# dgrzech/ir-sgmcmc

Measured on AMD Instinct MI355X. Metric: SG-MCMC transitions/sec (full _SGLD_transition), higher is better.
Workload: dtype f32; 1 GPU; 256^3 synthetic pair, SVF_3D 12 steps, GMM(K=4)/LCC(s=1) + virtual decimation, RegLoss_L2 w=1.4, Sobolev s=3, uniform noise 0.1, SGLD lr 0.4, Philox noise; init=identity, chains=1, parallelism=1 independent chain(s)

## Files before the change

### include/irsgmcmc.h

```cpp
#ifndef IRSGMCMC_H
#define IRSGMCMC_H

#include <stddef.h>
#include <stdint.h>

#ifdef __cplusplus
extern "C" {
#endif
#pragma GCC visibility push(default)

#define IRS_MAX_COMPONENTS 8
#define IRS_MAX_CHAINS 8
#define IRS_MAX_HALF_WIDTH 4
#define IRS_MAX_LABELS 64

enum { IRS_DATA_GMM_LCC = 0, IRS_DATA_SSD = 1 };
enum { IRS_REG_L2 = 0, IRS_REG_LOGNORMAL = 1, IRS_REG_STUDENT = 2, IRS_REG_LOGNORMAL_L2 = 3 };


int irs_perturb_smooth(const float* v, const float* sigma, const float* eps, float tau, const float* kernel, int s,
                       int C, int D, int H, int W, float* tmp, float* out, uint64_t seed, uint64_t iteration,
                       void* stream);

int irs_svf_exp_fwd(const float* v, float* steps, float* transformation, float* displacement, int no_steps, int C,
                    int D, int H, int W, void* stream);

int irs_svf_exp_bwd(const float* v, const float* steps, const float* g_last, float* scratch, float* g_v, int no_steps,
                    int C, int D, int H, int W, void* stream);

int irs_ffd_up(const float* v_cp, float* dense, float* tmp, int C, int D, int H, int W, int c0, int c1, int c2,
               void* stream);
int irs_ffd_adjoint(const float* g_dense, float* g_cp, float* tmp, int C, int D, int H, int W, int c0, int c1, int c2,
                    void* stream);

int irs_warp_fwd(const float* im, int Cim, const float* d_last, const float* unif, float alpha, float* warped, int C,
                 int D, int H, int W, uint64_t seed, uint64_t iteration, void* stream);
int irs_warp_bwd(const float* im, int Cim, const float* d_last, const float* unif, float alpha, const float* g_warped,
                 float* g_d, int C, int D, int H, int W, uint64_t seed, uint64_t iteration, void* stream);
int irs_warp_transformation(const float* im, int Cim, const float* transformation, float* warped, int C, int D, int H,
                            int W, void* stream);
int irs_warp_nearest_u8(const uint8_t* seg, int Cim, const float* transformation, uint8_t* out, int C, int D, int H,
                        int W, void* stream);
int irs_warp_nearest_i16(const int16_t* seg, int Cim, const float* transformation, int16_t* out, int C, int D, int H,
                         int W, void* stream);

int irs_lcc_normalise(const float* im, float* out, float* sigma_out, int s, int C, int D, int H, int W, void* stream);
int irs_lcc_map_fwd(const float* fhat, int Cf, const float* warped, float* z, float* sigma_m, int s, int C, int D,
                    int H, int W, void* stream);
int irs_lcc_map_bwd(const float* fhat, int Cf, const float* z, const float* sigma_m, const float* g_z, float* g_warped,
                    int s, int C, int D, int H, int W, void* stream);

int irs_reg_energy(const float* v, double* y_out, double* partials, int C, int D, int H, int W, void* stream);
size_t irs_reduce_scratch_doubles(void);
int irs_gradient_operator(const float* v, float* nabla, int transformation, int C, int D, int H, int W, void* stream);
int irs_log_det_jacobian(const float* transformation, float* log_det, long long* nan_count, int C, int D, int H, int W,
                         void* stream);

int irs_label_boxes(const int16_t* seg_fixed, int Cf, const int16_t* seg_moving, const int32_t* labels, int n_labels,
                    int32_t* boxes, int C, int D, int H, int W, void* stream);
// ... 211 lines not shown
```

### ir_sgmcmc_amd/_lib.py

```python
import ctypes as C
import os

import torch

_HERE = os.path.dirname(os.path.abspath(__file__))
LIB_PATH = os.environ.get('IRS_LIB') or os.path.join(_HERE, 'csrc', 'libirsgmcmc.so')

IRS_MAX_COMPONENTS = 8
IRS_MAX_CHAINS = 8
IRS_MAX_HALF_WIDTH = 4
IRS_MAX_LABELS = 64
IRS_DATA_GMM_LCC, IRS_DATA_SSD = 0, 1
IRS_REG_L2, IRS_REG_LOGNORMAL, IRS_REG_STUDENT, IRS_REG_LOGNORMAL_L2 = 0, 1, 2, 3


class IrsConfig(C.Structure):
    _fields_ = [
        ('dims', C.c_int32 * 3), ('cps', C.c_int32 * 3), ('no_chains', C.c_int32), ('no_steps', C.c_int32),
        ('sobolev_s', C.c_int32), ('sobolev_kernel', C.c_float * (2 * IRS_MAX_HALF_WIDTH + 1)),
        ('lr', C.c_float), ('uniform_alpha', C.c_float), ('virtual_decimation', C.c_int32),
        ('data_loss', C.c_int32), ('lcc_s', C.c_int32), ('gmm_components', C.c_int32), ('ssd_sigma', C.c_float),
        ('gmm_lr_log_std', C.c_float), ('gmm_lr_logits', C.c_float), ('gmm_lr_decay', C.c_float),
        ('adam_beta1', C.c_float), ('adam_beta2', C.c_float), ('adam_eps', C.c_float),
        ('scale_prior_loc', C.c_float), ('scale_prior_scale', C.c_float),
# ... 64 lines not shown
    _fields_ = [(n, C.c_int32) for n in ('kind', 'stage', 'k', 'lo0', 'hi0', 'lo1', 'hi1', 'in0', 'in1', 'reach', 'out', 'width', 'id')]


IRS_OP_LAUNCH, IRS_OP_EXCHANGE, IRS_OP_ALLREDUCE, IRS_OP_WAIT = range(4)
(IRS_SG_PERTURB, IRS_SG_COPY_V, IRS_SG_SMOOTH, IRS_SG_ENERGY, IRS_SG_EXP_FWD, IRS_SG_OUTPUTS, IRS_SG_WARP, IRS_SG_RESIDUAL, IRS_SG_STATS,
 IRS_SG_DATA_BWD, IRS_SG_WARP_BWD, IRS_SG_EXP_BWD, IRS_SG_UPDATE, IRS_SG_FFD_UP, IRS_SG_FFD_ADJ) = range(15)
IRS_SG_CHAIN_SCALAR, IRS_SG_REG_SCALAR, IRS_SG_FINALIZE = 32, 33, 34
(IRS_SB_V, IRS_SB_NOISY, IRS_SB_VS, IRS_SB_WARPED, IRS_SB_Z, IRS_SB_GM, IRS_SB_GRAD_A, IRS_SB_GRAD_B, IRS_SB_DENSE, IRS_SB_GRAD_C) = range(10)
IRS_SB_STEP0 = 16
IRS_COMM_ID_BYTES = 128
EXCHANGE_FN = C.CFUNCTYPE(C.c_int, C.c_void_p, C.POINTER(IrsXfer), C.c_int, C.c_void_p)
ALLREDUCE_FN = C.CFUNCTYPE(C.c_int, C.c_void_p, C.c_void_p, C.c_size_t, C.c_int, C.c_void_p)

_P, _I, _F, _U64 = C.c_void_p, C.c_int, C.c_float, C.c_uint64
_I32P = C.POINTER(C.c_int32)

SIGNATURES = {
    'irs_perturb_smooth': [_P, _P, _P, _F, _P, _I, _I, _I, _I, _I, _P, _P, _U64, _U64, _P],
    'irs_svf_exp_fwd': [_P, _P, _P, _P, _I, _I, _I, _I, _I, _P],
    'irs_svf_exp_bwd': [_P, _P, _P, _P, _P, _I, _I, _I, _I, _I, _P],
    'irs_ffd_up': [_P, _P, _P, _I, _I, _I, _I, _I, _I, _I, _P],
    'irs_ffd_adjoint': [_P, _P, _P, _I, _I, _I, _I, _I, _I, _I, _P],
    'irs_warp_fwd': [_P, _I, _P, _P, _F, _P, _I, _I, _I, _I, _U64, _U64, _P],
    'irs_warp_bwd': [_P, _I, _P, _P, _F, _P, _P, _I, _I, _I, _I, _U64, _U64, _P],
    'irs_warp_transformation': [_P, _I, _P, _P, _I, _I, _I, _I, _P],
    'irs_warp_nearest_u8': [_P, _I, _P, _P, _I, _I, _I, _I, _P],
    'irs_warp_nearest_i16': [_P, _I, _P, _P, _I, _I, _I, _I, _P],
    'irs_lcc_normalise': [_P, _P, _P, _I, _I, _I, _I, _I, _P],
    'irs_lcc_map_fwd': [_P, _I, _P, _P, _P, _I, _I, _I, _I, _I, _P],
    'irs_lcc_map_bwd': [_P, _I, _P, _P, _P, _P, _I, _I, _I, _I, _I, _P],
    'irs_reg_energy': [_P, _P, _P, _I, _I, _I, _I, _P],
    'irs_reduce_scratch_doubles': [],
    'irs_gradient_operator': [_P, _P, _I, _I, _I, _I, _I, _P],
    'irs_log_det_jacobian': [_P, _P, _P, _I, _I, _I, _I, _P],
    'irs_label_boxes': [_P, _I, _P, _I32P, _I, _P, _I, _I, _I, _I, _P],
    'irs_surface_distance_workspace': [_I32P, _I, _I, _I, _I, C.POINTER(C.c_size_t)],
    'irs_label_surface_distance': [_P, _I, _P, _I32P, _I, C.POINTER(C.c_float), _I32P, _P, C.c_size_t, _P, _P, _I, _I, _I, _I,
                                   _P],
    'irs_chain_moments_update': [_P, _I, _I, _I, _I, _I, _I, _P, _P, _P],
    'irs_split_rhat_workspace': [_I, _I, _I, _I, C.POINTER(C.c_size_t)],
    'irs_split_rhat': [_P, _P, _I, _I, _P, C.c_float, C.c_float, _P, _P, _P, C.c_size_t, _I, _I, _I, _P],
    'irs_chain_variogram_update': [_P, _I, _I, _I, _I, _I, _I, _P, _P, _P],
    'irs_split_ess_workspace': [_I, _I, _I, _I, C.POINTER(C.c_size_t)],
    'irs_split_ess': [_P, _P, _P, _I, _I, _I, _P, C.c_float, _P, _P, _P, _P, C.c_size_t, _I, _I, _I, _P],
    'irs_create': [C.POINTER(IrsConfig), C.POINTER(_P)],
    'irs_destroy': [_P],
# ... 90 lines not shown
```

### ir_sgmcmc_amd/csrc/api.hip

```cpp
#include <math.h>
#include <stdarg.h>
#include <stdio.h>
#include <stdlib.h>
#include <string.h>

#include <algorithm>
#include <mutex>
#include <new>
#include <vector>

#include "comm.h"
#include "ctx.h"

using namespace irs;

namespace irs {
thread_local char g_err[512] = "";

int fail(const char* fmt, ...) {
    va_list ap;
    va_start(ap, fmt);
    vsnprintf(g_err, sizeof(g_err), fmt, ap);
    va_end(ap);
    return 1;
// ... 4 lines not shown

static int env_or(const char* name, int dflt) {
    const char* v = getenv(name);
    return v && *v ? atoi(v) : dflt;
}

static Knobs knobs_from_env() {
    Knobs k;
    k.predict_variants = env_or("IRS_PREDICT_VARIANTS", k.predict_variants);
    k.run_ahead = env_or("IRS_RUN_AHEAD", k.run_ahead);
    k.fuse_warp_bwd = env_or("IRS_FUSE_WARP_BWD", k.fuse_warp_bwd);
    k.energy_in_update = env_or("IRS_ENERGY_IN_UPDATE", k.energy_in_update);
    k.fuse_noise = env_or("IRS_FUSE_NOISE", k.fuse_noise);
    k.recover = env_or("IRS_RECOVER", k.recover);
    k.fwd_rows1 = env_or("IRS_FWD_ROWS1", k.fwd_rows1);
    k.coarse_box = env_or("IRS_COARSE_BOX", k.coarse_box);
    k.lds_from = env_or("IRS_LDS_FROM", k.lds_from);
    k.seg_fit = env_or("IRS_SEG_FIT", k.seg_fit);
    k.fwd_pf = env_or("IRS_FWD_PF", k.fwd_pf);
    k.fwd_z2 = env_or("IRS_FWD_Z2", k.fwd_z2);
    k.tile_box = env_or("IRS_TILE_BOX", k.tile_box);
    k.fwd_r2_rows1 = env_or("IRS_FWD_R2_ROWS1", k.fwd_r2_rows1);
    k.ps_rows = env_or("IRS_PS_ROWS", k.ps_rows);
    const char* tile = getenv("IRS_SOBOLEV_TILE");
    if (tile && *tile) k.sobolev_tile = tile[0] == 'b' ? 2 : (tile[0] == 's' ? 1 : atoi(tile));
    k.march_seg = env_or("IRS_MARCH_SEG", k.march_seg);
    k.march_seg_fwd = env_or("IRS_MARCH_SEG_FWD", k.march_seg_fwd);
    k.swz_run = env_or("IRS_SWZ_RUN", k.swz_run);
    k.seg_min_blocks = env_or("IRS_SEG_MIN_BLOCKS", k.seg_min_blocks);
    k.seg_min_len = env_or("IRS_SEG_MIN_LEN", k.seg_min_len);
    k.sobolev_seg = env_or("IRS_SOBOLEV_SEG", k.sobolev_seg);
    k.lcc_seg = env_or("IRS_LCC_SEG", k.lcc_seg);
    k.stats_seg = env_or("IRS_STATS_SEG", k.stats_seg);
    k.update_seg = env_or("IRS_UPDATE_SEG", k.update_seg);
    k.slab_split = env_or("IRS_SLAB_SPLIT", k.slab_split);
    k.slab_buffers = env_or("IRS_SLAB_BUFFERS", k.slab_buffers);
    k.slab_exact = env_or("IRS_SLAB_EXACT", k.slab_exact);
    k.slab_force_h = env_or("IRS_SLAB_FORCE_H", k.slab_force_h);
    k.launch_log = env_or("IRS_LAUNCH_LOG", k.launch_log);
    k.chain_overlap = env_or("IRS_CHAIN_OVERLAP", k.chain_overlap);
    k.data_batch = env_or("IRS_DATA_BATCH", k.data_batch);
    return k;
}

Knobs& global_knobs() {
    static Knobs k = knobs_from_env();
// ... 20 lines not shown
            (double)steps / (double)(steps - run_in > 0 ? steps - run_in : 1));
}

static int g_live_contexts = 0;
void context_born() { ++g_live_contexts; }
void context_gone() { --g_live_contexts; }

enum { KN_CTX = 0, KN_GLOBAL = 1, KN_LAYOUT = 2 };

int knob_set(Knobs& k, const char* name, int value, bool on_context) {
    struct Entry {
        const char* name;
        int Knobs::*field;
        int scope;
    };
    static const Entry table[] = {
        {"predict_variants", &Knobs::predict_variants, KN_CTX}, {"run_ahead", &Knobs::run_ahead, KN_CTX}, {"fuse_warp_bwd", &Knobs::fuse_warp_bwd, KN_CTX},
        {"energy_in_update", &Knobs::energy_in_update, KN_CTX}, {"fuse_noise", &Knobs::fuse_noise, KN_CTX}, {"recover", &Knobs::recover, KN_CTX},
        {"chain_overlap", &Knobs::chain_overlap, KN_CTX}, {"data_batch", &Knobs::data_batch, KN_CTX}, {"slab_split", &Knobs::slab_split, KN_CTX}, {"slab_buffers", &Knobs::slab_buffers, KN_CTX}, {"slab_exact", &Knobs::slab_exact, KN_CTX}, {"slab_force_h", &Knobs::slab_force_h, KN_CTX},
        {"fwd_rows1", &Knobs::fwd_rows1, KN_GLOBAL}, {"coarse_box", &Knobs::coarse_box, KN_GLOBAL}, {"lds_from", &Knobs::lds_from, KN_GLOBAL},
        {"fwd_pf", &Knobs::fwd_pf, KN_GLOBAL}, {"fwd_z2", &Knobs::fwd_z2, KN_GLOBAL}, {"tile_box", &Knobs::tile_box, KN_GLOBAL}, {"fwd_r2_rows1", &Knobs::fwd_r2_rows1, KN_GLOBAL}, {"sobolev_tile", &Knobs::sobolev_tile, KN_GLOBAL},
        {"march_seg", &Knobs::march_seg, KN_GLOBAL}, {"march_seg_fwd", &Knobs::march_seg_fwd, KN_GLOBAL}, {"swz_run", &Knobs::swz_run, KN_GLOBAL},
        {"sobolev_seg", &Knobs::sobolev_seg, KN_GLOBAL}, {"ps_rows", &Knobs::ps_rows, KN_GLOBAL}, {"launch_log", &Knobs::launch_log, KN_GLOBAL},
        {"seg_fit", &Knobs::seg_fit, KN_LAYOUT}, {"seg_min_blocks", &Knobs::seg_min_blocks, KN_LAYOUT}, {"seg_min_len", &Knobs::seg_min_len, KN_LAYOUT},
        {"lcc_seg", &Knobs::lcc_seg, KN_LAYOUT}, {"stats_seg", &Knobs::stats_seg, KN_LAYOUT}, {"update_seg", &Knobs::update_seg, KN_LAYOUT},
    };
    if (!name) return fail("irs_option_set: null name");
    for (const Entry& e : table)
        if (!strcmp(e.name, name)) {
            if (on_context && e.scope != KN_CTX)
                return fail("irs_option_set: '%s' is a process-wide switch (the launchers read it at every launch): set it with ctx == NULL", name);
            if (!on_context && e.scope == KN_LAYOUT && g_live_contexts > 0 && k.*(e.field) != value)
                return fail("irs_option_set: '%s' sizes the partial-sum layout of a context at creation; %d context(s) are alive -- set it before irs_create", name, g_live_contexts);
            k.*(e.field) = value;
            return 0;
        }
    return fail("irs_option_set: unknown option '%s'", name);
}
}

namespace {

bool dims_ok(int C, int D, int H, int W) {
    return C >= 1 && D >= 2 && H >= 2 && W >= 2 && (int64_t)D * H * W < ((int64_t)1 << 30);
}

// ... 179 lines not shown
               void* stream) {
    if (!v_cp || !dense || !tmp || !dims_ok(C, D, H, W) || c0 < 1 || c1 < 1 || c2 < 1 || c0 > 8 || c1 > 8 || c2 > 8)
        return fail("irs_ffd_up: bad arguments");
    const Vol vol = make_vol(D, H, W);
    const int G[3] = {control_points(D, c0), control_points(H, c1), control_points(W, c2)};
    const SplineTaps spl[3] = {make_spline(c0), make_spline(c1), make_spline(c2)};
    ffd_up(v_cp, dense, tmp, C, vol, G, spl, (hipStream_t)stream);
    LAUNCH_CHECK();
    return 0;
}

int irs_ffd_adjoint(const float* g_dense, float* g_cp, float* tmp, int C, int D, int H, int W, int c0, int c1, int c2,
                    void* stream) {
    if (!g_dense || !g_cp || !tmp || !dims_ok(C, D, H, W) || c0 < 1 || c1 < 1 || c2 < 1 || c0 > 8 || c1 > 8 || c2 > 8)
        return fail("irs_ffd_adjoint: bad arguments");
    const Vol vol = make_vol(D, H, W);
    const int G[3] = {control_points(D, c0), control_points(H, c1), control_points(W, c2)};
    const SplineTaps spl[3] = {make_spline(c0), make_spline(c1), make_spline(c2)};
    ffd_adjoint(g_dense, g_cp, tmp, C, vol, G, spl, (hipStream_t)stream);
    LAUNCH_CHECK();
    return 0;
}

int irs_warp_fwd(const float* im, int Cim, const float* d_last, const float* unif, float alpha, float* warped, int C,
                 int D, int H, int W, uint64_t seed, uint64_t iteration, void* stream) {
    if (!im || !d_last || !warped || !dims_ok(C, D, H, W) || (Cim != 1 && Cim != C)) return fail("irs_warp_fwd: bad arguments");
    hipStream_t st = (hipStream_t)stream;
    const Vol vol = make_vol(D, H, W);
    Lin lin;
    if (cached_lin(D, H, W, st, &lin)) return fail("irs_warp_fwd: identity grid allocation failed");
    launch_warp_fwd(im, Cim == 1 ? 0 : vol.V, d_last, unif, alpha, warped, nullptr, 0, C, vol, lin, seed, iteration, nullptr, st);
    LAUNCH_CHECK();
    return 0;
}

int irs_warp_bwd(const float* im, int Cim, const float* d_last, const float* unif, float alpha, const float* g_warped,
                 float* g_d, int C, int D, int H, int W, uint64_t seed, uint64_t iteration, void* stream) {
    if (!im || !d_last || !g_warped || !g_d || !dims_ok(C, D, H, W) || (Cim != 1 && Cim != C))
        return fail("irs_warp_bwd: bad arguments");
    hipStream_t st = (hipStream_t)stream;
    const Vol vol = make_vol(D, H, W);
    Lin lin;
    if (cached_lin(D, H, W, st, &lin)) return fail("irs_warp_bwd: identity grid allocation failed");
    launch_warp_bwd(im, Cim == 1 ? 0 : vol.V, d_last, unif, alpha, g_warped, g_d, C, vol, lin, seed, iteration, nullptr, st);
    LAUNCH_CHECK();
    return 0;
// ... 590 lines not shown
            launch_sobolev_march(c->tmpA, vs, c->sob, C * 3, c->volv, have_dmax0 ? c->dmax : nullptr, cfg.no_steps, st);
        }
    }
    const float* dense = vs;
    if (c->ffd) {
        const int G[3] = {c->volv.D, c->volv.H, c->volv.W};
        ffd_up(vs, c->dense, c->tmpA, C, c->vol, G, c->spl, st);
        dense = c->dense;
    }
    if (timed) HIP_TRY(hipEventRecord(c->ev[1], st));
    const int64_t field = (int64_t)c->C * 3 * c->vol.V;
    const Lin lin = c->lin.lin();
    if (!have_dmax0) launch_field_absmax(dense, true, cfg.no_steps, c->dmax, C, c->vol, st);
    for (int k = 0; k < cfg.no_steps; ++k) {
        const float* in = k == 0 ? dense : c->steps + (int64_t)(k - 1) * field;
        float* out = c->steps + (int64_t)k * field;
        launch_exp_step_fwd_march(in, out, k == 0, cfg.no_steps, C, c->vol, lin, c->dmax + (int64_t)k * c->C * 4,
                                  c->dmax + (int64_t)(k + 1) * c->C * 4, predicted_small(c, k), fwd_lay(c, k), st);
    }
    if (timed) HIP_TRY(hipEventRecord(c->ev[2], st));
    const float* d_last = c->steps + (int64_t)(cfg.no_steps - 1) * field;
    const float alpha = with_jitter ? cfg.uniform_alpha : 0.0f;
    launch_warp_fwd(io->moving_im, io->moving_chains == 1 ? 0 : c->vol.V, d_last, io->unif, alpha, warped, gradm, 1, C, c->vol, lin,
                    cfg.seed, 0, it, st);
    if (cfg.data_loss == IRS_DATA_GMM_LCC)
        launch_lcc_fwd_march(c->fhat, c->fhat_chains == 1 ? 0 : c->vol.V, warped, z, c->sigM, cfg.lcc_s, C, c->vol, st);
    else
        launch_residual_ssd(io->fixed_im, io->fixed_chains == 1 ? 0 : c->vol.V, warped, z, C, c->vol, st);
    LAUNCH_CHECK();
    return 0;
}

int irs_gmm_init(irs_ctx* c, const irs_io* io, const float* v_sample, int warm_up, void* stream) {
    if (check_io(c, io, "irs_gmm_init")) return 1;
    if (c->cfg.data_loss != IRS_DATA_GMM_LCC) return 0;
    hipStream_t st = (hipStream_t)stream;
    const size_t bytes = (size_t)3 * c->volv.V * sizeof(float);
    if (v_sample) HIP_TRY(hipMemcpyAsync(c->tmpB, v_sample, bytes, hipMemcpyDeviceToDevice, st));
    else HIP_TRY(hipMemsetAsync(c->tmpB, 0, bytes, st));
    if (forward_pass(c, io, c->tmpB, false, false, c->vs, c->warped, c->z, nullptr, 1, st, 0)) return 1;
    launch_masked_moments(c->z, io->mask, c->stat_partials, c->vol, st);
    launch_gmm_init_from_moments(c->state, c->stat_partials, stats_blocks(c->vol), c->dcfg, st);
    launch_stats(c->cfg.virtual_decimation, c->z, io->mask, c->state, c->stat_partials, c->vol, st, c->dcfg.K);
    launch_chain_scalar(c->state, c->stat_partials, stats_blocks(c->vol), 0, 1, c->dcfg, st);
    for (int i = 0; i < warm_up; ++i) {
        launch_stats(0, c->z, io->mask, c->state, c->stat_partials, c->vol, st, c->dcfg.K);
        launch_chain_scalar(c->state, c->stat_partials, stats_blocks(c->vol), 0, 2, c->dcfg, st);
// ... 233 lines not shown
```

### ir_sgmcmc_amd/csrc/common.h

```cpp
#pragma once
#include <hip/hip_runtime.h>
#include <math.h>
#include <stdint.h>
#include <stdlib.h>

#include "../../include/irsgmcmc.h"

namespace irs {

constexpr int kBlock = 256;
constexpr int kWave = 64;
constexpr int kMaxPartialBlocks = 2048;

struct Vol {
    int D, H, W;
    int64_t V;
    int z0, nz;
    int z0b, nzb;
    int64_t Vg;
};

__host__ __device__ inline Vol make_vol(int D, int H, int W) {
    return Vol{D, H, W, (int64_t)D * H * W, 0, D, 0, 0, (int64_t)D * H * W};
}
// ... 43 lines not shown
    int run_ahead = 2;
    int fuse_warp_bwd = 1;
    int energy_in_update = 1;
    int fuse_noise = 1;
    int recover = 1;
    int fwd_rows1 = -1;
    int lds_from = 3;
    int fwd_r2_rows1 = 1;
    int fwd_z2 = 0;
    int tile_box = 1;
    int fwd_pf = 2;
    int seg_fit = 1;
    int coarse_box = 1;
    int sobolev_tile = 0;
    int ps_rows = 0;
    int march_seg = 0, march_seg_fwd = 0, swz_run = -1, seg_min_blocks = 0, seg_min_len = 0;
    int sobolev_seg = 0, lcc_seg = 0, stats_seg = 0, update_seg = 0;
    int slab_buffers = 3;
    int slab_split = 1;
    int slab_exact = 0;
    int slab_force_h = 0;
    int data_batch = 1;
    int chain_overlap = 0;
    int launch_log = 0;
};
Knobs& global_knobs();
int knob_set(Knobs& k, const char* name, int value, bool on_context);

inline int pick_seg_len(int nz, int64_t tiles_per_layer, int min_len, int forced, int64_t want_blocks = 1024) {
    if (forced > 0) return forced;
    const Knobs& kn = global_knobs();
    if (kn.seg_min_len > 0) min_len = kn.seg_min_len;
    const int64_t want = kn.seg_min_blocks > 0 ? kn.seg_min_blocks : want_blocks;
    int len = 32;
    while (len > min_len && tiles_per_layer * ((nz + len - 1) / len) < want) len >>= 1;
    return len < 1 ? 1 : len;
}

inline int pick_seg_len_fit(int nz, int nzb, int64_t tiles_per_layer, int min_len, int run_in, int64_t resident, int forced,
                            int max_len = 32) {
    if (forced > 0) return forced;
    const int longest = nz > nzb ? nz : nzb;
    int best = 32;
    int64_t best_cost = -1;
    for (int len = max_len; len >= min_len; --len) {
        if (len > longest && len != 32) continue;
// ... 206 lines not shown
```

### ir_sgmcmc_amd/csrc/field_kernels.hip

```cpp
#include "kernels.h"
#include "warp_device.h"

namespace irs {

__global__ __launch_bounds__(kBlock) void perturb_kernel(const float* __restrict__ v, const float* __restrict__ sigma,
                                                         const float* __restrict__ eps, float amp,
                                                         float* __restrict__ out, Vol vol, uint64_t seed,
                                                         uint64_t iteration, const uint64_t* dev_iter, int npair) {
    const int x = blockIdx.x * 64 + (threadIdx.x & 63), y = blockIdx.y * 4 + (threadIdx.x >> 6);
    const int chain = blockIdx.z / npair;
    const int za = 2 * ((vol.z0 >> 1) + (int)blockIdx.z - chain * npair);
    if (x >= vol.W || y >= vol.H) return;
    const int64_t V = vol.V, HW = (int64_t)vol.H * vol.W;
    const int64_t voxa = ((int64_t)za * vol.H + y) * vol.W + x;
    float n[2][3];
    if (!eps) {
        const uint64_t it = dev_iter ? *dev_iter : iteration;
        const uint64_t idx = (uint64_t)chain * (uint64_t)vol.Vg + (uint64_t)voxa;
        const U4 r = philox4x32_10(U4{(uint32_t)idx, (uint32_t)(idx >> 32), (uint32_t)it, 0x5347u ^ (uint32_t)(it >> 32)},
                                   (uint32_t)seed, (uint32_t)(seed >> 32));
        uint32_t w[6];
        split21(r, w);
        box_muller21(w[0], w[1], n[0][0], n[0][1]);
        box_muller21(w[2], w[3], n[0][2], n[1][0]);
// ... 117 lines not shown
        vox[h] = ((int64_t)z * vol.H + y) * vol.W + x;
        grid_point(d, unif, jt, cb3, chain, vox[h], vol, lin, x, y, z, g[h]);
    }
#pragma unroll
    for (int h = 0; h < NV; ++h) wv[h] = gradm ? warp_sample<true>(src, g[h], vol, gm[h]) : warp_sample<false>(src, g[h], vol, gm[h]);
#pragma unroll
    for (int h = 0; h < NV; ++h) {
        if (y0 + 4 * h >= vol.H) continue;
        out[(int64_t)chain * vol.V + vox[h]] = wv[h];
        if (gradm) {
            if (gradm_aos) {
                typedef float f3v __attribute__((ext_vector_type(3)));
                const f3v v = {gm[h][0], gm[h][1], gm[h][2]};
                __builtin_memcpy(gradm + cb3 + vox[h] * 3, &v, 12);
            } else {
                gradm[cb3 + vox[h]] = gm[h][0];
                gradm[cb3 + vol.V + vox[h]] = gm[h][1];
                gradm[cb3 + 2 * vol.V + vox[h]] = gm[h][2];
            }
        }
    }
}

void launch_warp_fwd(const float* im, int64_t im_stride, const float* d, const float* unif, float alpha, float* out,
                     float* gradm, int gradm_aos, int C, Vol vol, Lin lin, uint64_t seed, uint64_t iteration,
                     const uint64_t* dev_iteration, hipStream_t st) {
    const dim3 grid((unsigned)((vol.W + 63) / 64), (unsigned)((vol.H + 4 * IRS_WARP_NV - 1) / (4 * IRS_WARP_NV)), (unsigned)(vol.nz * C));
    hipLaunchKernelGGL(warp_fwd_kernel, grid, dim3(kBlock), 0, st, im, im_stride, d, unif,
                       make_jitter(alpha, vol, seed, iteration, dev_iteration), out, gradm, gradm_aos, vol, lin);
}

__global__ __launch_bounds__(kBlock) void warp_bwd_kernel(const float* __restrict__ im, int64_t im_stride,
                                                          const float* __restrict__ d, const float* __restrict__ unif,
                                                          Jitter jt, const float* __restrict__ gw,
                                                          float* __restrict__ gd, Vol vol, Lin lin) {
    IRS_VOXEL(vol, chain, x, y, z, vox);
    const int64_t cb3 = (int64_t)chain * 3 * vol.V;
    float g[3];
    grid_point(d, unif, jt, cb3, chain, vox, vol, lin, x, y, z, g);
    const AxisTap tx = axis_tap(g[0], vol.W), ty = axis_tap(g[1], vol.H), tz = axis_tap(g[2], vol.D);
    const float* src = im + (int64_t)chain * im_stride;
    float gix = 0.0f, giy = 0.0f, giz = 0.0f;
#pragma unroll
    for (int cz = 0; cz < 2; ++cz)
#pragma unroll
        for (int cy = 0; cy < 2; ++cy) {
            const int64_t rowoff = ((int64_t)(cz ? tz.i1 : tz.i0) * vol.H + (cy ? ty.i1 : ty.i0)) * vol.W;
#pragma unroll
            for (int cx = 0; cx < 2; ++cx) {
                const float wx = cx ? tx.w1 : tx.w0, wy = cy ? ty.w1 : ty.w0, wz = cz ? tz.w1 : tz.w0;
                const float val = src[rowoff + (cx ? tx.i1 : tx.i0)];
                gix += (cx ? val : -val) * (wy * wz);
// ... 183 lines not shown
```

### ir_sgmcmc_amd/csrc/kernels.h

```cpp
#pragma once
#include "common.h"

namespace irs {

struct Taps {
    float k[2 * IRS_MAX_HALF_WIDTH + 1];
    int s;
};

struct SplineTaps {
    float k[32];
    int cps;
};

struct LinTables {
    float* dev = nullptr;
    int D = 0, H = 0, W = 0;
    Lin lin() const { return Lin{dev, dev + W, dev + W + H}; }
};
int ensure_lin_tables(LinTables& t, int D, int H, int W, hipStream_t st);
int cached_lin(int D, int H, int W, hipStream_t st, Lin* out);

void launch_perturb(const float* v, const float* sigma, const float* eps, float amp, float* out, int C, Vol vol,
                    uint64_t seed, uint64_t iteration, const uint64_t* dev_iteration, hipStream_t st);
void launch_svf_outputs(const float* d, float* transformation, float* displacement, int C, Vol vol, Lin lin,
                        hipStream_t st);
void launch_warp_fwd(const float* im, int64_t im_stride, const float* d, const float* unif, float alpha, float* out,
                     float* gradm, int gradm_aos, int C, Vol vol, Lin lin, uint64_t seed, uint64_t iteration,
                     const uint64_t* dev_iteration, hipStream_t st);
void launch_warp_bwd(const float* im, int64_t im_stride, const float* d, const float* unif, float alpha,
                     const float* g_warped, float* g_d, int C, Vol vol, Lin lin, uint64_t seed, uint64_t iteration,
                     const uint64_t* dev_iteration, hipStream_t st);
void launch_warp_transformation(const float* im, int64_t im_stride, const float* t, float* out, int C, Vol vol,
                                hipStream_t st);
void launch_warp_nearest_u8(const uint8_t* im, int64_t im_stride, const float* t, uint8_t* out, int C, Vol vol,
                            hipStream_t st);
void launch_warp_nearest_i16(const int16_t* im, int64_t im_stride, const float* t, int16_t* out, int C, Vol vol,
                             hipStream_t st);
void launch_ffd_axis(const float* in, float* out, const SplineTaps& taps, bool adjoint, int64_t outer, int n_in,
                     int n_out, int64_t inner, hipStream_t st, int w_lo = 0, int w_n = -1, int store_lo = 0, int store_n = -1);
void launch_scale_channels(const float* in, float* out, float s0, float s1, float s2, int C, Vol vol, hipStream_t st);

void launch_exp_step_fwd_march(const float* din, float* dout, bool prescale, int no_steps, int C, Vol vol, Lin lin,
                               const unsigned* dmax_in, unsigned* dmax_out, bool only_r1, int lay, hipStream_t st);
void launch_exp_step_bwd_march(const float* G, const float* dk, float* gout, bool prescale, int no_steps, int C, Vol vol,
                               Lin lin, const unsigned* dmax, int max_radius, bool r2_owns_rest, const float* gscale, int lay,
                               hipEvent_t after_primary, hipStream_t st);
size_t coarse_minmax_bytes(Vol vol, int C);
void launch_exp_step_bwd_lds(const float* G, const float* dk, float* gout, bool prescale, int no_steps, int C, Vol vol,
                             Lin lin, const unsigned* dmax, int halo, int gather_radius, const float* gscale, int lay,
                             float* cmm, hipStream_t st);
void launch_field_absmax(const float* d, bool prescale, int no_steps, unsigned* dmax, int C, Vol vol, hipStream_t st);
// ... 80 lines not shown
```

### ir_sgmcmc_amd/csrc/warp_device.h

```cpp
#pragma once
#include <math.h>

#include "common.h"

namespace irs {

struct Jitter {
    float alpha;
    float nm1[3];
    float rnm1[3];
    uint64_t seed, iteration;
    const uint64_t* dev_iter;
};

inline Jitter make_jitter(float alpha, Vol vol, uint64_t seed, uint64_t iteration, const uint64_t* dev_iter) {
    Jitter j;
    j.alpha = alpha;
    j.nm1[0] = (float)(vol.W - 1);
    j.nm1[1] = (float)(vol.H - 1);
    j.nm1[2] = (float)(vol.D - 1);
    for (int c = 0; c < 3; ++c) j.rnm1[c] = exact_rcp(j.nm1[c]);
    j.seed = seed;
    j.iteration = iteration;
    j.dev_iter = dev_iter;
// ... 3 lines not shown
__device__ __forceinline__ void jitter_point(float (&g)[3], const float* __restrict__ unif, const Jitter& jt, int64_t cb3,
                                             int chain, int64_t vox, int64_t V, int64_t Vg) {
    if (jt.alpha <= 0.0f) return;
    float u[3];
    if (unif) {
        u[0] = unif[cb3 + vox];
        u[1] = unif[cb3 + V + vox];
        u[2] = unif[cb3 + 2 * V + vox];
    } else {
        const uint64_t it = jt.dev_iter ? *jt.dev_iter : jt.iteration;
        const uint64_t idx = (uint64_t)chain * (uint64_t)Vg + (uint64_t)vox;
        const U2 r = philox2x32_10(U2{(uint32_t)idx, (uint32_t)(idx >> 32) | ((uint32_t)it << 4)}, key_mix(jt.seed, it, 0x554Eu));
        u[0] = u01_21(r.x >> 11);
        u[1] = u01_21(r.y >> 11);
        u[2] = u01_21((r.x & 0x7FFu) | ((r.y & 0x3FFu) << 11));
    }
#pragma unroll
    for (int c = 0; c < 3; ++c) {
        const float nz = __fadd_rn(__fmul_rn(-2.0f * jt.alpha, u[c]), jt.alpha);
        g[c] = __fadd_rn(g[c], div_exact(__fmul_rn(nz, 2.0f), jt.nm1[c], jt.rnm1[c]));
    }
}

template <bool WANT_GRAD>
__device__ __forceinline__ float warp_sample(const float* __restrict__ src, const float (&g)[3], const Vol vol, float (&gm)[3]) {
    const AxisTap tx = axis_tap(g[0], vol.W), ty = axis_tap(g[1], vol.H), tz = axis_tap(g[2], vol.D);
    float acc = 0.0f, gix = 0.0f, giy = 0.0f, giz = 0.0f;
    const unsigned hw = (unsigned)(vol.H * vol.W);
    const unsigned offz[2] = {(unsigned)tz.i0 * hw, (unsigned)tz.i0 * hw + (tz.i1 != tz.i0 ? hw : 0u)};
    const unsigned offy[2] = {(unsigned)ty.i0 * (unsigned)vol.W, (unsigned)ty.i0 * (unsigned)vol.W + (ty.i1 != ty.i0 ? (unsigned)vol.W : 0u)};
#pragma unroll
    for (int cz = 0; cz < 2; ++cz)
#pragma unroll
        for (int cy = 0; cy < 2; ++cy) {
            const unsigned rowoff = offz[cz] + offy[cy];
#pragma unroll
            for (int cx = 0; cx < 2; ++cx) {
                const float wx = cx ? tx.w1 : tx.w0, wy = cy ? ty.w1 : ty.w0, wz = cz ? tz.w1 : tz.w0;
                const float val = *reinterpret_cast<const float*>(reinterpret_cast<const char*>(src) + (size_t)((rowoff + (unsigned)(cx ? tx.i1 : tx.i0)) * 4u));
                acc = __fadd_rn(acc, __fmul_rn(val, __fmul_rn(__fmul_rn(wx, wy), wz)));
                if (WANT_GRAD) {
                    gix += (cx ? val : -val) * (wy * wz);
                    giy += (cy ? val : -val) * (wx * wz);
                    giz += (cz ? val : -val) * (wx * wy);
                }
            }
        }
    if (WANT_GRAD) {
        gm[0] = tx.gmul * gix;
        gm[1] = ty.gmul * giy;
        gm[2] = tz.gmul * giz;
    }
    return acc;
}

struct WarpArgs {
    const float* im;
    int64_t im_stride;
    const float* unif;
    Jitter jt;
    float* warped;
    float* gradm;
    int gradm_aos;
};

}
```

### ir_sgmcmc_amd/ops.py

```python
import ctypes as C
import math

import numpy as np
import torch

from . import _lib as L


def _dims5(t, ch=None):
    if t.dim() != 5 or (ch is not None and t.shape[1] != ch):
        raise L.IrsError(f'expected a (C,{ch if ch else "ch"},D,H,W) tensor, got {tuple(t.shape)}')
    return t.shape[0], t.shape[2], t.shape[3], t.shape[4]


def sobolev_kernel_1d(s, lam):
    n = 2 * s + 1
    lap = -2.0 * np.eye(n) + np.eye(n, k=1) + np.eye(n, k=-1)
    e = np.zeros(n)
    e[s] = 1.0
    col = np.linalg.solve(np.eye(n) - lam * lap, e)
    return (col / col.sum()).astype(np.float32)


def control_grid_size(dims, cps):
# ... 48 lines not shown
                           L.stream_ptr()))
    return dense


def ffd_adjoint(g_dense, cps):
    lib = L.load()
    Cn, D, H, W = _dims5(g_dense, 3)
    G = control_grid_size((D, H, W), cps)
    g_cp = torch.empty((Cn, 3, *G), device=g_dense.device, dtype=torch.float32)
    tmp = torch.empty((2, Cn, 3, D, H, W), device=g_dense.device, dtype=torch.float32)
    L.check(lib.irs_ffd_adjoint(L.dev_ptr(g_dense.contiguous(), torch.float32), L.dev_ptr(g_cp), L.dev_ptr(tmp), Cn, D, H,
                                W, *cps, L.stream_ptr()))
    return g_cp


def warp_displacement(im, d_last, unif=None, alpha=0.0, seed=0, iteration=0):
    lib = L.load()
    Cn, D, H, W = _dims5(d_last, 3)
    out = torch.empty((Cn, 1, D, H, W), device=d_last.device, dtype=torch.float32)
    L.check(lib.irs_warp_fwd(L.dev_ptr(im, torch.float32), im.shape[0], L.dev_ptr(d_last, torch.float32),
                             L.dev_ptr(unif, torch.float32, True), float(alpha), L.dev_ptr(out), Cn, D, H, W, seed,
                             iteration, L.stream_ptr()))
    return out


def warp_displacement_bwd(im, d_last, g_warped, unif=None, alpha=0.0, seed=0, iteration=0):
    lib = L.load()
    Cn, D, H, W = _dims5(d_last, 3)
    g_d = torch.empty_like(d_last)
    L.check(lib.irs_warp_bwd(L.dev_ptr(im, torch.float32), im.shape[0], L.dev_ptr(d_last, torch.float32),
                             L.dev_ptr(unif, torch.float32, True), float(alpha),
                             L.dev_ptr(g_warped.contiguous(), torch.float32), L.dev_ptr(g_d), Cn, D, H, W, seed, iteration,
                             L.stream_ptr()))
    return g_d


def warp(im, transformation):
    lib = L.load()
    Cn, D, H, W = _dims5(transformation, 3)
    if im.dim() != 5 or im.shape[1] != 1 or im.shape[0] not in (1, Cn) or tuple(im.shape[2:]) != (D, H, W):
        raise L.IrsError(f'image shape {tuple(im.shape)} does not match transformation {tuple(transformation.shape)}')
    t = L.dev_ptr(transformation, torch.float32)
    if im.dtype == torch.float32:
        out = torch.empty((Cn, 1, D, H, W), device=im.device, dtype=torch.float32)
        L.check(lib.irs_warp_transformation(L.dev_ptr(im), im.shape[0], t, L.dev_ptr(out), Cn, D, H, W, L.stream_ptr()))
        return out
# ... 169 lines not shown
```

Baseline: 231.6 transitions/s.

## Add z-marching shared-memory ring warp forward kernel with displacement-bound fallback

After: 232.8 transitions/s, median of 6. No clear change (+0.5%).

```diff
diff --git a/include/irsgmcmc.h b/include/irsgmcmc.h
--- a/include/irsgmcmc.h
+++ b/include/irsgmcmc.h
@@ -35,6 +35,9 @@
 
 int irs_warp_fwd(const float* im, int Cim, const float* d_last, const float* unif, float alpha, float* warped, int C,
                  int D, int H, int W, uint64_t seed, uint64_t iteration, void* stream);
+int irs_warp_fwd_window(const float* im, int Cim, const float* d_last, const float* unif, float alpha, float* warped,
+                        float* gradm, int C, int D, int H, int W, int z0, int nz, uint64_t seed, uint64_t iteration,
+                        void* stream);
 int irs_warp_bwd(const float* im, int Cim, const float* d_last, const float* unif, float alpha, const float* g_warped,
                  float* g_d, int C, int D, int H, int W, uint64_t seed, uint64_t iteration, void* stream);
 int irs_warp_transformation(const float* im, int Cim, const float* transformation, float* warped, int C, int D, int H,
diff --git a/ir_sgmcmc_amd/_lib.py b/ir_sgmcmc_amd/_lib.py
--- a/ir_sgmcmc_amd/_lib.py
+++ b/ir_sgmcmc_amd/_lib.py
@@ -110,6 +110,7 @@
     'irs_ffd_up': [_P, _P, _P, _I, _I, _I, _I, _I, _I, _I, _P],
     'irs_ffd_adjoint': [_P, _P, _P, _I, _I, _I, _I, _I, _I, _I, _P],
     'irs_warp_fwd': [_P, _I, _P, _P, _F, _P, _I, _I, _I, _I, _U64, _U64, _P],
+    'irs_warp_fwd_window': [_P, _I, _P, _P, _F, _P, _P, _I, _I, _I, _I, _I, _I, _U64, _U64, _P],
     'irs_warp_bwd': [_P, _I, _P, _P, _F, _P, _P, _I, _I, _I, _I, _U64, _U64, _P],
     'irs_warp_transformation': [_P, _I, _P, _P, _I, _I, _I, _I, _P],
     'irs_warp_nearest_u8': [_P, _I, _P, _P, _I, _I, _I, _I, _P],
diff --git a/ir_sgmcmc_amd/csrc/api.hip b/ir_sgmcmc_amd/csrc/api.hip
--- a/ir_sgmcmc_amd/csrc/api.hip
+++ b/ir_sgmcmc_amd/csrc/api.hip
@@ -50,6 +50,8 @@
     k.tile_box = env_or("IRS_TILE_BOX", k.tile_box);
     k.fwd_r2_rows1 = env_or("IRS_FWD_R2_ROWS1", k.fwd_r2_rows1);
     k.ps_rows = env_or("IRS_PS_ROWS", k.ps_rows);
+    k.warp_march = env_or("IRS_WARP_MARCH", k.warp_march);
+    k.warp_seg = env_or("IRS_WARP_SEG", k.warp_seg);
     const char* tile = getenv("IRS_SOBOLEV_TILE");
     if (tile && *tile) k.sobolev_tile = tile[0] == 'b' ? 2 : (tile[0] == 's' ? 1 : atoi(tile));
     k.march_seg = env_or("IRS_MARCH_SEG", k.march_seg);
@@ -116,6 +118,7 @@
         {"fwd_pf", &Knobs::fwd_pf, KN_GLOBAL}, {"fwd_z2", &Knobs::fwd_z2, KN_GLOBAL}, {"tile_box", &Knobs::tile_box, KN_GLOBAL}, {"fwd_r2_rows1", &Knobs::fwd_r2_rows1, KN_GLOBAL}, {"sobolev_tile", &Knobs::sobolev_tile, KN_GLOBAL},
         {"march_seg", &Knobs::march_seg, KN_GLOBAL}, {"march_seg_fwd", &Knobs::march_seg_fwd, KN_GLOBAL}, {"swz_run", &Knobs::swz_run, KN_GLOBAL},
         {"sobolev_seg", &Knobs::sobolev_seg, KN_GLOBAL}, {"ps_rows", &Knobs::ps_rows, KN_GLOBAL}, {"launch_log", &Knobs::launch_log, KN_GLOBAL},
+        {"warp_march", &Knobs::warp_march, KN_GLOBAL}, {"warp_seg", &Knobs::warp_seg, KN_GLOBAL},
         {"seg_fit", &Knobs::seg_fit, KN_LAYOUT}, {"seg_min_blocks", &Knobs::seg_min_blocks, KN_LAYOUT}, {"seg_min_len", &Knobs::seg_min_len, KN_LAYOUT},
         {"lcc_seg", &Knobs::lcc_seg, KN_LAYOUT}, {"stats_seg", &Knobs::stats_seg, KN_LAYOUT}, {"update_seg", &Knobs::update_seg, KN_LAYOUT},
     };
@@ -341,6 +344,20 @@
     return 0;
 }
 
+int irs_warp_fwd_window(const float* im, int Cim, const float* d_last, const float* unif, float alpha, float* warped,
+                        float* gradm, int C, int D, int H, int W, int z0, int nz, uint64_t seed, uint64_t iteration,
+                        void* stream) {
+    if (!im || !d_last || !warped || !dims_ok(C, D, H, W) || (Cim != 1 && Cim != C) || z0 < 0 || nz < 0 || z0 + nz > D)
+        return fail("irs_warp_fwd_window: bad arguments");
+    hipStream_t st = (hipStream_t)stream;
+    const Vol vol = window(make_vol(D, H, W), z0, z0 + nz);
+    Lin lin;
+    if (cached_lin(D, H, W, st, &lin)) return fail("irs_warp_fwd_window: identity grid allocation failed");
+    launch_warp_fwd(im, Cim == 1 ? 0 : vol.V, d_last, unif, alpha, warped, gradm, 1, C, vol, lin, seed, iteration, nullptr, st);
+    LAUNCH_CHECK();
+    return 0;
+}
+
 int irs_warp_fwd(const float* im, int Cim, const float* d_last, const float* unif, float alpha, float* warped, int C,
                  int D, int H, int W, uint64_t seed, uint64_t iteration, void* stream) {
     if (!im || !d_last || !warped || !dims_ok(C, D, H, W) || (Cim != 1 && Cim != C)) return fail("irs_warp_fwd: bad arguments");
@@ -977,7 +994,7 @@
     const float* d_last = c->steps + (int64_t)(cfg.no_steps - 1) * field;
     const float alpha = with_jitter ? cfg.uniform_alpha : 0.0f;
     launch_warp_fwd(io->moving_im, io->moving_chains == 1 ? 0 : c->vol.V, d_last, io->unif, alpha, warped, gradm, 1, C, c->vol, lin,
-                    cfg.seed, 0, it, st);
+                    cfg.seed, 0, it, st, c->dmax + (int64_t)cfg.no_steps * c->C * 4);
     if (cfg.data_loss == IRS_DATA_GMM_LCC)
         launch_lcc_fwd_march(c->fhat, c->fhat_chains == 1 ? 0 : c->vol.V, warped, z, c->sigM, cfg.lcc_s, C, c->vol, st);
     else
diff --git a/ir_sgmcmc_amd/csrc/common.h b/ir_sgmcmc_amd/csrc/common.h
--- a/ir_sgmcmc_amd/csrc/common.h
+++ b/ir_sgmcmc_amd/csrc/common.h
@@ -89,6 +89,8 @@
     int slab_force_h = 0;
     int data_batch = 1;
     int chain_overlap = 0;
+    int warp_march = -1;
+    int warp_seg = 0;
     int launch_log = 0;
 };
 Knobs& global_knobs();
diff --git a/ir_sgmcmc_amd/csrc/field_kernels.hip b/ir_sgmcmc_amd/csrc/field_kernels.hip
--- a/ir_sgmcmc_amd/csrc/field_kernels.hip
+++ b/ir_sgmcmc_amd/csrc/field_kernels.hip
@@ -163,12 +163,192 @@
     }
 }
 
+#ifndef IRS_WTY
+#define IRS_WTY 4
+#define IRS_WROWS 1
+#endif
+constexpr int WTX = 64, WTY = IRS_WTY, WROWS = IRS_WROWS, kWarpBlock = WTX * WTY / WROWS;
+template <int R>
+struct MarchW {
+    static constexpr int NS = 2 * R + 2;
+    static constexpr int PX = WTX + 2 * R, PY = WTY + 2 * R, PN = PX * PY;
+    static constexpr int NIT = (PN + kWarpBlock - 1) / kWarpBlock;
+};
+
+template <int R, bool GRAD>
+__global__ __launch_bounds__(kWarpBlock) void warp_fwd_march_kernel(const float* __restrict__ im, int64_t im_stride,
+                                                                    const float* __restrict__ d, const float* __restrict__ unif,
+                                                                    Jitter jt, float* __restrict__ out, float* __restrict__ gradm,
+                                                                    int gradm_aos, Vol vol, Lin lin, int seg_len, int nseg,
+                                                                    int swz_run, dim3 tiles, const unsigned* __restrict__ dmax) {
+    using M = MarchW<R>;
+    constexpr int NS = M::NS, PX = M::PX, PY = M::PY, PN = M::PN, NIT = M::NIT;
+    __shared__ float ring[NS * PN];
+    const int tile_ = xcd_swizzle_runs((int)blockIdx.x, (int)(tiles.x * tiles.y * tiles.z), swz_run);
+    const int tbx = tile_ % tiles.x, tby = (tile_ / tiles.x) % tiles.y, tbz = tile_ / (tiles.x * tiles.y);
+    const int chain = tbz / nseg, seg = tbz % nseg;
+    const int ox = tbx * WTX, oy = tby * WTY;
+    int z0, z1;
+    seg_range(vol, seg, seg_len, z0, z1);
+    const int64_t V = vol.V, cb3 = (int64_t)chain * 3 * V;
+    const int HW = vol.H * vol.W;
+    const float* __restrict__ src = im + (int64_t)chain * im_stride;
+    if (jt.dev_iter) {
+        jt.iteration = *jt.dev_iter;
+        jt.dev_iter = nullptr;
+    }
+    const int lx = threadIdx.x % WTX, ly0 = threadIdx.x / WTX;
+    const int x = ox + lx, xc = min(x, vol.W - 1);
+    const float linx = lin.x[xc];
+    float liny[WROWS];
+    int yoff[WROWS];
+#pragma unroll
+    for (int j = 0; j < WROWS; ++j) {
+        const int yc = min(oy + ly0 + j * (WTY / WROWS), vol.H - 1);
+        liny[j] = lin.y[yc];
+        yoff[j] = yc * vol.W + xc;
+    }
+    int sxy[NIT];
+#pragma unroll
+    for (int it = 0; it < NIT; ++it) {
+        const int i = threadIdx.x + it * kWarpBlock;
+        const int cx = min(max(ox - R + i % PX, 0), vol.W - 1), cy = min(max(oy - R + i / PX, 0), vol.H - 1);
+        sxy[it] = i < PN ? cy * vol.W + cx : -1;
+    }
+    float pre[NIT];
+    auto prefetch = [&](int s) {
+        const float* __restrict__ pl = src + (int64_t)min(max(s, 0), vol.D - 1) * HW;
+#pragma unroll
+        for (int it = 0; it < NIT; ++it)
+            if (sxy[it] >= 0) pre[it] = pl[(unsigned)sxy[it]];
+    };
+    float dn[WROWS][3], linz_n = 0.0f;
+    auto load_d = [&](int zo) {
+        const int64_t pb = cb3 + (int64_t)zo * HW;
+#pragma unroll
+        for (int j = 0; j < WROWS; ++j)
+#pragma unroll
+            for (int c = 0; c < 3; ++c) dn[j][c] = d[pb + c * V + yoff[j]];
+        linz_n = lin.z[zo];
+    };
+    auto store = [&](int64_t vox, float wv, const float (&gm)[3]) {
+        out[(int64_t)chain * V + vox] = wv;
+        if (GRAD) {
+            if (gradm_aos) {
+                typedef float f3v __attribute__((ext_vector_type(3)));
+                const f3v v = {gm[0], gm[1], gm[2]};
+                __builtin_memcpy(gradm + cb3 + vox * 3, &v, 12);
+            } else {
+                gradm[cb3 + vox] = gm[0];
+                gradm[cb3 + V + vox] = gm[1];
+                gradm[cb3 + 2 * V + vox] = gm[2];
+            }
+        }
+    };
+    if (dmax && fmaxf(fmaxf(__uint_as_float(dmax[chain * 4 + 0]), __uint_as_float(dmax[chain * 4 + 1])), __uint_as_float(dmax[chain * 4 + 2])) +
+                        fmaxf(jt.alpha, 0.0f) >= 2.0f * R) {
+        for (int zo = z0; zo < z1; ++zo) {
+            const float linz = lin.z[zo];
+#pragma unroll
+            for (int j = 0; j < WROWS; ++j) {
+                const int y = oy + ly0 + j * (WTY / WROWS);
+                if (x >= vol.W || y >= vol.H) continue;
+                const int64_t vox = (int64_t)zo * HW + (y * vol.W + x);
+                float g[3] = {__fadd_rn(linx, d[cb3 + vox]), __fadd_rn(liny[j], d[cb3 + V + vox]), __fadd_rn(linz, d[cb3 + 2 * V + vox])};
+                jitter_point(g, unif, jt, cb3, chain, vox, V, vol.Vg);
+                float gm[3];
+                const float wv = warp_sample<GRAD>(src, g, vol, gm);
+                store(vox, wv, gm);
+            }
+        }
+        return;
+    }
+    const int sbase = z0 - R, slast = z1 - 1 + R;
+    prefetch(sbase);
+    for (int sb = sbase; sb <= slast; sb += NS) {
+#pragma unroll 1
+        for (int PH = 0; PH < NS; ++PH) {
+            const int s = sb + PH;
+            if (s > slast) break;
+            __builtin_amdgcn_s_waitcnt(0x0F70);
+#pragma unroll
+            for (int it = 0; it < NIT; ++it)
+                if (sxy[it] >= 0) ring[PH * PN + threadIdx.x + it * kWarpBlock] = pre[it];
+            float dc[WROWS][3];
+#pragma unroll
+            for (int j = 0; j < WROWS; ++j)
+#pragma unroll
+                for (int c = 0; c < 3; ++c) dc[j][c] = dn[j][c];
+            const float linz = linz_n;
+            const int zo = s - R;
+            if (zo + 1 >= z0 && zo + 1 < z1) load_d(zo + 1);
+            if (s + 1 <= slast) prefetch(s + 1);
+            __syncthreads();
+            if (zo < z0 || zo >= z1) continue;
+#pragma unroll
+            for (int j = 0; j < WROWS; ++j) {
+                const int y = oy + ly0 + j * (WTY / WROWS);
+                if (x >= vol.W || y >= vol.H) continue;
+                const int64_t vox = (int64_t)zo * HW + (y * vol.W + x);
+                float g[3] = {__fadd_rn(linx, dc[j][0]), __fadd_rn(liny[j], dc[j][1]), __fadd_rn(linz, dc[j][2])};
+                jitter_point(g, unif, jt, cb3, chain, vox, V, vol.Vg);
+                const AxisTap tx = axis_tap(g[0], vol.W), ty = axis_tap(g[1], vol.H), tz = axis_tap(g[2], vol.D);
+                const int bx0 = tx.i0 - (ox - R), by0 = ty.i0 - (oy - R), rel = tz.i0 - zo;
+                const bool in_ring = (unsigned)bx0 < (unsigned)(PX - 1) && (unsigned)by0 < (unsigned)(PY - 1) && rel >= -R && rel < R;
+                float gm[3], wv;
+                auto ring_sample = [&]() {
+                    int sl0 = ((PH - 2 * R + 2 * NS) % NS) * PN, sl1 = ((PH - 2 * R + 1 + 2 * NS) % NS) * PN;
+#pragma unroll
+                    for (int q = -R + 1; q < R; ++q) {
+                        sl0 = rel == q ? ((PH - R + q + 2 * NS) % NS) * PN : sl0;
+                        sl1 = rel == q ? ((PH - R + q + 1 + 2 * NS) % NS) * PN : sl1;
+                    }
+                    const int off = by0 * PX + bx0;
+                    return warp_taps<GRAD>(tx, ty, tz, [&](int cz, int cy, int cx) { return ring[(cz ? sl1 : sl0) + off + cy * PX + cx]; }, gm);
+                };
+                if (__all(in_ring)) wv = ring_sample();
+                else if (in_ring) wv = ring_sample();
+                else wv = warp_taps<GRAD>(tx, ty, tz, [&](int cz, int cy, int cx) {
+                    return src[((int64_t)(cz ? tz.i1 : tz.i0) * vol.H + (cy ? ty.i1 : ty.i0)) * vol.W + (cx ? tx.i1 : tx.i0)];
+                }, gm);
+                store(vox, wv, gm);
+            }
+        }
+    }
+}
+
+static bool warp_march_on(int C, const Vol& vol) {
+    const int k = global_knobs().warp_march;
+    return k >= 0 ? k != 0 : (int64_t)C * vol.nz * vol.H * vol.W >= ((int64_t)1 << 22);
+}
+
 void launch_warp_fwd(const float* im, int64_t im_stride, const float* d, const float* unif, float alpha, float* out,
                      float* gradm, int gradm_aos, int C, Vol vol, Lin lin, uint64_t seed, uint64_t iteration,
-                     const uint64_t* dev_iteration, hipStream_t st) {
+                     const uint64_t* dev_iteration, hipStream_t st, const unsigned* dmax) {
+    const Jitter jt = make_jitter(alpha, vol, seed, iteration, dev_iteration);
+    if (vol.nz <= 0 || C <= 0) return;
+    if (warp_march_on(C, vol)) {
+        Vol w = window(vol, vol.z0, vol.z0 + vol.nz);
+        const int64_t per_layer = (int64_t)((vol.W + WTX - 1) / WTX) * ((vol.H + WTY - 1) / WTY) * C;
+        static int cache = 0;
+        const int64_t res = resident_blocks((const void*)warp_fwd_march_kernel<1, true>, kWarpBlock, &cache);
+        const int seg_len = pick_seg_len_fit(w.nz, 0, per_layer, 8, 2, res > 0 ? res : 2048, global_knobs().warp_seg);
+        const int nseg = vol_nseg(w, seg_len);
+        const dim3 tiles((unsigned)((vol.W + WTX - 1) / WTX), (unsigned)((vol.H + WTY - 1) / WTY), (unsigned)(nseg * C));
+        const int total = (int)(tiles.x * tiles.y * tiles.z);
+        const int swz_env = global_knobs().swz_run;
+        const int swz_run = swz_env >= 0 ? swz_env : (int)tiles.x;
+        if (global_knobs().launch_log) {
+            static int cache_l = 0;
+            log_launch("warp_fwd_march_kernel<R=1>", WTX, WTY, total, kWarpBlock, seg_len, 2, w.nz, C,
+                       resident_blocks((const void*)warp_fwd_march_kernel<1, true>, kWarpBlock, &cache_l));
+        }
+        if (gradm) hipLaunchKernelGGL((warp_fwd_march_kernel<1, true>), dim3(total), dim3(kWarpBlock), 0, st, im, im_stride, d, unif, jt, out, gradm, gradm_aos, w, lin, seg_len, nseg, swz_run, tiles, dmax);
+        else hipLaunchKernelGGL((warp_fwd_march_kernel<1, false>), dim3(total), dim3(kWarpBlock), 0, st, im, im_stride, d, unif, jt, out, gradm, gradm_aos, w, lin, seg_len, nseg, swz_run, tiles, dmax);
+        return;
+    }
     const dim3 grid((unsigned)((vol.W + 63) / 64), (unsigned)((vol.H + 4 * IRS_WARP_NV - 1) / (4 * IRS_WARP_NV)), (unsigned)(vol.nz * C));
-    hipLaunchKernelGGL(warp_fwd_kernel, grid, dim3(kBlock), 0, st, im, im_stride, d, unif,
-                       make_jitter(alpha, vol, seed, iteration, dev_iteration), out, gradm, gradm_aos, vol, lin);
+    hipLaunchKernelGGL(warp_fwd_kernel, grid, dim3(kBlock), 0, st, im, im_stride, d, unif, jt, out, gradm, gradm_aos, vol, lin);
 }
 
 __global__ __launch_bounds__(kBlock) void warp_bwd_kernel(const float* __restrict__ im, int64_t im_stride,
diff --git a/ir_sgmcmc_amd/csrc/kernels.h b/ir_sgmcmc_amd/csrc/kernels.h
--- a/ir_sgmcmc_amd/csrc/kernels.h
+++ b/ir_sgmcmc_amd/csrc/kernels.h
@@ -27,7 +27,7 @@
                         hipStream_t st);
 void launch_warp_fwd(const float* im, int64_t im_stride, const float* d, const float* unif, float alpha, float* out,
                      float* gradm, int gradm_aos, int C, Vol vol, Lin lin, uint64_t seed, uint64_t iteration,
-                     const uint64_t* dev_iteration, hipStream_t st);
+                     const uint64_t* dev_iteration, hipStream_t st, const unsigned* dmax = nullptr);
 void launch_warp_bwd(const float* im, int64_t im_stride, const float* d, const float* unif, float alpha,
                      const float* g_warped, float* g_d, int C, Vol vol, Lin lin, uint64_t seed, uint64_t iteration,
                      const uint64_t* dev_iteration, hipStream_t st);
diff --git a/ir_sgmcmc_amd/csrc/warp_device.h b/ir_sgmcmc_amd/csrc/warp_device.h
--- a/ir_sgmcmc_amd/csrc/warp_device.h
+++ b/ir_sgmcmc_amd/csrc/warp_device.h
@@ -49,22 +49,17 @@
     }
 }
 
-template <bool WANT_GRAD>
-__device__ __forceinline__ float warp_sample(const float* __restrict__ src, const float (&g)[3], const Vol vol, float (&gm)[3]) {
-    const AxisTap tx = axis_tap(g[0], vol.W), ty = axis_tap(g[1], vol.H), tz = axis_tap(g[2], vol.D);
+template <bool WANT_GRAD, typename Load>
+__device__ __forceinline__ float warp_taps(const AxisTap& tx, const AxisTap& ty, const AxisTap& tz, Load&& load, float (&gm)[3]) {
     float acc = 0.0f, gix = 0.0f, giy = 0.0f, giz = 0.0f;
-    const unsigned hw = (unsigned)(vol.H * vol.W);
-    const unsigned offz[2] = {(unsigned)tz.i0 * hw, (unsigned)tz.i0 * hw + (tz.i1 != tz.i0 ? hw : 0u)};
-    const unsigned offy[2] = {(unsigned)ty.i0 * (unsigned)vol.W, (unsigned)ty.i0 * (unsigned)vol.W + (ty.i1 != ty.i0 ? (unsigned)vol.W : 0u)};
 #pragma unroll
     for (int cz = 0; cz < 2; ++cz)
 #pragma unroll
-        for (int cy = 0; cy < 2; ++cy) {
-            const unsigned rowoff = offz[cz] + offy[cy];
+        for (int cy = 0; cy < 2; ++cy)
 #pragma unroll
             for (int cx = 0; cx < 2; ++cx) {
                 const float wx = cx ? tx.w1 : tx.w0, wy = cy ? ty.w1 : ty.w0, wz = cz ? tz.w1 : tz.w0;
-                const float val = *reinterpret_cast<const float*>(reinterpret_cast<const char*>(src) + (size_t)((rowoff + (unsigned)(cx ? tx.i1 : tx.i0)) * 4u));
+                const float val = load(cz, cy, cx);
                 acc = __fadd_rn(acc, __fmul_rn(val, __fmul_rn(__fmul_rn(wx, wy), wz)));
                 if (WANT_GRAD) {
                     gix += (cx ? val : -val) * (wy * wz);
@@ -72,7 +67,6 @@
                     giz += (cz ? val : -val) * (wx * wy);
                 }
             }
-        }
     if (WANT_GRAD) {
         gm[0] = tx.gmul * gix;
         gm[1] = ty.gmul * giy;
@@ -81,14 +75,15 @@
     return acc;
 }
 
-struct WarpArgs {
-    const float* im;
-    int64_t im_stride;
-    const float* unif;
-    Jitter jt;
-    float* warped;
-    float* gradm;
-    int gradm_aos;
-};
+template <bool WANT_GRAD>
+__device__ __forceinline__ float warp_sample(const float* __restrict__ src, const float (&g)[3], const Vol vol, float (&gm)[3]) {
+    const AxisTap tx = axis_tap(g[0], vol.W), ty = axis_tap(g[1], vol.H), tz = axis_tap(g[2], vol.D);
+    const unsigned hw = (unsigned)(vol.H * vol.W);
+    const unsigned offz[2] = {(unsigned)tz.i0 * hw, (unsigned)tz.i0 * hw + (tz.i1 != tz.i0 ? hw : 0u)};
+    const unsigned offy[2] = {(unsigned)ty.i0 * (unsigned)vol.W, (unsigned)ty.i0 * (unsigned)vol.W + (ty.i1 != ty.i0 ? (unsigned)vol.W : 0u)};
+    return warp_taps<WANT_GRAD>(tx, ty, tz, [&](int cz, int cy, int cx) {
+        return *reinterpret_cast<const float*>(reinterpret_cast<const char*>(src) + (size_t)((offz[cz] + offy[cy] + (unsigned)(cx ? tx.i1 : tx.i0)) * 4u));
+    }, gm);
+}
 
 }
diff --git a/ir_sgmcmc_amd/ops.py b/ir_sgmcmc_amd/ops.py
--- a/ir_sgmcmc_amd/ops.py
+++ b/ir_sgmcmc_amd/ops.py
@@ -94,6 +94,21 @@
                              L.dev_ptr(unif, torch.float32, True), float(alpha), L.dev_ptr(out), Cn, D, H, W, seed,
                              iteration, L.stream_ptr()))
     return out
+
+
+def warp_displacement_window(im, d_last, z0=0, nz=None, unif=None, alpha=0.0, seed=0, iteration=0, grad=True, out=None, gradm=None):
+    lib = L.load()
+    Cn, D, H, W = _dims5(d_last, 3)
+    nz = D - z0 if nz is None else nz
+    if out is None:
+        out = torch.zeros((Cn, 1, D, H, W), device=d_last.device, dtype=torch.float32)
+    if grad and gradm is None:
+        gradm = torch.zeros((Cn, D, H, W, 3), device=d_last.device, dtype=torch.float32)
+    L.check(lib.irs_warp_fwd_window(L.dev_ptr(im, torch.float32), im.shape[0], L.dev_ptr(d_last, torch.float32),
+                                    L.dev_ptr(unif, torch.float32, True), float(alpha), L.dev_ptr(out),
+                                    L.dev_ptr(gradm) if grad else None, Cn, D, H, W, int(z0), int(nz), seed, iteration,
+                                    L.stream_ptr()))
+    return (out, gradm) if grad else out
 
 
 def warp_displacement_bwd(im, d_last, g_warped, unif=None, alpha=0.0, seed=0, iteration=0):
```
